# tigarcia/firedancer

Measured on AMD Instinct MI355X. Metric: ed25519 verifies/sec at 1/8 GPUs; % INT32 VALU roofline; p99 batch latency, higher is better.
Workload: dtype int32

## Files before the change

### firedancer_amd/csrc/fd25519_half.h

```cpp
#ifndef FD25519_HALF_H
#define FD25519_HALF_H

#include <stdint.h>

#ifndef FD_HALF_FN
#define FD_HALF_FN static inline
#endif

#define FD_HALF_BITS 131
#define FD_HALF_DBITS_MAX 151
#define FD_HALF_TW   5
#ifndef FD_HALF_LEHMER_MARGIN
#define FD_HALF_LEHMER_MARGIN 0
#endif

#define FD_HALF_N8L {0xe7ae9f68u, 0xc09318d2u, 0x17bce6b2u, 0xa6f7cef5u, 0u, 0u, 0u, 0x80000000u}

template <int N>
FD_HALF_FN int fd_half_bitlen(const uint32_t (&x)[N]) {
  int r = 0;
#pragma unroll
  for (int i = 0; i < N; i++)
    if (x[i]) r = 32 * i + 32 - __builtin_clz(x[i]);
  return r;
}

FD_HALF_FN uint64_t fd_half_shr64(const uint32_t (&x)[8], int s) {
  const int w = s >> 5, sh = s & 31;
  uint32_t x0 = 0u, x1 = 0u, x2 = 0u;
#pragma unroll
  for (int i = 0; i < 8; i++) {
    x0 = i == w ? x[i] : x0;
    x1 = i == w + 1 ? x[i] : x1;
    x2 = i == w + 2 ? x[i] : x2;
  }
  const uint64_t lo = (((uint64_t)x1 << 32) | x0) >> sh;
  const uint64_t hi = (((uint64_t)x2 << 32) | x1) >> sh;
  return (lo & 0xffffffffu) | (hi << 32);
}

FD_HALF_FN int fd_half_lt(const uint32_t (&a)[8], const uint32_t (&b)[8]) {
  int r = 0;
#pragma unroll
  for (int i = 0; i < 8; i++) r = a[i] != b[i] ? (a[i] < b[i]) : r;
  return r;
}

template <int N>
FD_HALF_FN void fd_half_mul_small(uint32_t (&out)[N], const uint32_t (&x)[N], uint64_t m) {
  const uint64_t m0 = m & 0xffffffffu, m1 = m >> 32;
  uint64_t c = 0;
#pragma unroll
  for (int i = 0; i < N; i++) {
    const uint64_t t = (uint64_t)x[i] * m0 + c;
    out[i] = (uint32_t)t;
    c = t >> 32;
  }
  c = 0;
#pragma unroll
  for (int i = 0; i + 1 < N; i++) {
    const uint64_t t = (uint64_t)x[i] * m1 + out[i + 1] + c;
    out[i + 1] = (uint32_t)t;
    c = t >> 32;
  }
}

template <int N>
FD_HALF_FN void fd_half_lin(uint32_t (&out)[N], const uint32_t (&x)[N], const uint32_t (&y)[N], int64_t A,
                            int64_t B) {
  uint32_t px[N], py[N];
  fd_half_mul_small<N>(px, x, (uint64_t)(A < 0 ? -A : A));
  fd_half_mul_small<N>(py, y, (uint64_t)(B < 0 ? -B : B));
  const uint32_t fx = A < 0 ? 0xffffffffu : 0u, fy = B < 0 ? 0xffffffffu : 0u;
  uint64_t c = (uint64_t)(A < 0) + (uint64_t)(B < 0);
#pragma unroll
  for (int i = 0; i < N; i++) {
    const uint64_t t = (uint64_t)(px[i] ^ fx) + (uint64_t)(py[i] ^ fy) + c;
    out[i] = (uint32_t)t;
    c = t >> 32;
  }
}

FD_HALF_FN void fd_half_step(uint32_t (&a)[8], const uint32_t (&b)[8], uint32_t (&ta)[FD_HALF_TW],
                             const uint32_t (&tb)[FD_HALF_TW], uint64_t q) {
  uint32_t p[8], pt[FD_HALF_TW];
  fd_half_mul_small<8>(p, b, q);
  fd_half_mul_small<FD_HALF_TW>(pt, tb, q);
  uint64_t br = 0;
#pragma unroll
  for (int i = 0; i < 8; i++) {
    const uint64_t t = (uint64_t)a[i] - p[i] - br;
    a[i] = (uint32_t)t;
    br = (t >> 63) & 1u;
  }
  br = 0;
#pragma unroll
  for (int i = 0; i < FD_HALF_TW; i++) {
    const uint64_t t = (uint64_t)ta[i] - pt[i] - br;
    ta[i] = (uint32_t)t;
    br = (t >> 63) & 1u;
  }
}

FD_HALF_FN uint64_t fd_half_quot(const uint32_t (&a)[8], const uint32_t (&b)[8]) {
  const int la = fd_half_bitlen<8>(a);
  const int s = la > 52 ? la - 52 : 0;
  const uint64_t ah = fd_half_shr64(a, s), bh = fd_half_shr64(b, s);
  const double r = (double)ah / (double)(bh + 1u) * (1.0 - 0x1p-40);
  const uint64_t q = (uint64_t)r;
  return q ? q : 1u;
}

FD_HALF_FN void fd_half_swap(uint32_t (&a)[8], uint32_t (&b)[8], uint32_t (&ta)[FD_HALF_TW],
                             uint32_t (&tb)[FD_HALF_TW], int cond) {
#pragma unroll
  for (int i = 0; i < 8; i++) {
    const uint32_t x = a[i], y = b[i];
    a[i] = cond ? y : x;
    b[i] = cond ? x : y;
  }
#pragma unroll
  for (int i = 0; i < FD_HALF_TW; i++) {
    const uint32_t x = ta[i], y = tb[i];
    ta[i] = cond ? y : x;
    tb[i] = cond ? x : y;
  }
}

FD_HALF_FN void fd_half_single(uint32_t (&a)[8], uint32_t (&b)[8], uint32_t (&ta)[FD_HALF_TW],
                               uint32_t (&tb)[FD_HALF_TW]) {
  fd_half_step(a, b, ta, tb, fd_half_quot(a, b));
  fd_half_swap(a, b, ta, tb, fd_half_lt(a, b));
}

#ifndef FD_HALF_RCP
#define FD_HALF_RCP(y) (1.0 / (y))
#endif
FD_HALF_FN double fd_half_fdiv(double x, double y) {
  double r = FD_HALF_RCP(y);
  r = __builtin_fma(r, __builtin_fma(-y, r, 1.0), r);
  double q = __builtin_floor(x * r);
#pragma unroll
  for (int i = 0; i < 2; i++) {
    const double rem = __builtin_fma(-q, y, x);
    q = rem < 0.0 ? q - 1.0 : (rem >= y ? q + 1.0 : q);
  }
  return q;
}

#ifndef FD_HALF_RCPF
#define FD_HALF_RCPF(y) (1.0f / (y))
#endif
FD_HALF_FN double fd_half_fdiv32(double x, double y) {
  double q = __builtin_floor((double)((float)x * FD_HALF_RCPF((float)y)));
  double rem = __builtin_fma(-q, y, x);
  q = rem < 0.0 ? q - 1.0 : (rem >= y ? q + 1.0 : q);
  rem = __builtin_fma(-q, y, x);
  return (rem >= 0.0 && rem < y) ? q : -1.0;
}

FD_HALF_FN double fd_half_fdiv20(double x, double y) {
  const double e = (double)((float)x * FD_HALF_RCPF((float)y));
  double q = __builtin_floor(e);
  const double rem = __builtin_fma(-q, y, x);
  q = rem < 0.0 ? q - 1.0 : (rem >= y ? q + 1.0 : q);
  return e < 0x1p20 ? q : -1.0;
}

#ifndef FD_HALF_INNER
#define FD_HALF_INNER 4
#endif
#if FD_HALF_INNER >= 3
#define FD_HALF_QUOT(x, y) fd_half_fdiv20((x), (y))
#elif FD_HALF_INNER == 2
#define FD_HALF_QUOT(x, y) fd_half_fdiv32((x), (y))
#else
#define FD_HALF_QUOT(x, y) fd_half_fdiv((x), (y))
#endif

FD_HALF_FN int fd_half_abs(uint32_t (&mag)[FD_HALF_TW], const uint32_t (&x)[FD_HALF_TW]) {
  const int neg = (int)(x[FD_HALF_TW - 1] >> 31);
  const uint32_t f = neg ? 0xffffffffu : 0u;
  uint64_t c = (uint64_t)neg;
#pragma unroll
  for (int i = 0; i < FD_HALF_TW; i++) {
    const uint64_t t = (uint64_t)(x[i] ^ f) + c;
    mag[i] = (uint32_t)t;
    c = t >> 32;
  }
  return neg;
}

FD_HALF_FN int fd_half_scalars(const uint32_t (&k)[8], uint32_t (&c)[FD_HALF_TW], uint32_t (&dmag)[FD_HALF_TW],
                               int* dneg, int dbits) {
  uint32_t a[8] = FD_HALF_N8L, b[8];
  uint32_t ta[FD_HALF_TW] = {0u, 0u, 0u, 0u, 0u}, tb[FD_HALF_TW] = {1u, 0u, 0u, 0u, 0u};
#pragma unroll
  for (int i = 0; i < 8; i++) b[i] = k[i];
  int ok = 1, it = 0;

  while (fd_half_bitlen<8>(b) > FD_HALF_BITS + FD_HALF_LEHMER_MARGIN) {
    if (++it > 200) { ok = 0; break; }
    const int s = fd_half_bitlen<8>(a) - 52;
    double uh = (double)fd_half_shr64(a, s), vh = (double)fd_half_shr64(b, s);
    const int fl = FD_HALF_BITS + FD_HALF_LEHMER_MARGIN - s;
    const double floor_v = fl > 0 ? (double)((uint64_t)1 << (fl < 62 ? fl : 62)) : 0.0;
    double Af = 1.0, Bf = 0.0, Cf = 0.0, Df = 1.0;
    for (int inner = 0; inner < 64; inner++) {
      const double x1 = uh + Af, y1 = vh + Cf, x2 = uh + Bf, y2 = vh + Df;
#if FD_HALF_INNER == 0
      if (!(y1 > 0.0 && y2 > 0.0 && x1 >= 0.0 && x2 >= 0.0)) break;
      const double q = fd_half_fdiv(x1, y1);
      if (q != fd_half_fdiv(x2, y2)) break;
      const double nv = __builtin_fma(-q, vh, uh);
      if (nv < floor_v) break;
#elif FD_HALF_INNER == 4
      const bool valid = (y1 > 0.0) & (y2 > 0.0) & (x1 >= 0.0) & (x2 >= 0.0);
      const double q = fd_half_fdiv20(x1, y1), q2 = fd_half_fdiv20(x2, y2);
      const double nv = __builtin_fma(-q, vh, uh);
      const double nC = __builtin_fma(-q, Cf, Af), nD = __builtin_fma(-q, Df, Bf);
      const bool ok1 = valid & (q >= 0.0) & (q == q2) & (nv >= floor_v);
      const double x1b = vh + Cf, y1b = nv + nC, x2b = vh + Df, y2b = nv + nD;
      const bool validb = (y1b > 0.0) & (y2b > 0.0) & (x1b >= 0.0) & (x2b >= 0.0);
      const double qb = fd_half_fdiv20(x1b, y1b), q2b = fd_half_fdiv20(x2b, y2b);
      const double nvb = __builtin_fma(-qb, nv, vh);
      const double nCb = __builtin_fma(-qb, nC, Cf), nDb = __builtin_fma(-qb, nD, Df);
      const bool ok2 = validb & (qb >= 0.0) & (qb == q2b) & (nvb >= floor_v);
      if (!(ok1 & ok2)) {
        if (ok1) { Af = Cf; Cf = nC; Bf = Df; Df = nD; uh = vh; vh = nv; }
        break;
      }
      Af = nC; Cf = nCb; Bf = nD; Df = nDb;
      uh = nv; vh = nvb;
      inner++;
      continue;
#elif FD_HALF_INNER == 3
      const bool valid = (y1 > 0.0) & (y2 > 0.0) & (x1 >= 0.0) & (x2 >= 0.0);
      const double q = FD_HALF_QUOT(x1, y1), q2 = FD_HALF_QUOT(x2, y2);
      const double nv = __builtin_fma(-q, vh, uh);
      const double nC = __builtin_fma(-q, Cf, Af), nD = __builtin_fma(-q, Df, Bf);
      if (!(valid & (q >= 0.0) & (q == q2) & (nv >= floor_v))) break;
      Af = Cf; Cf = nC; Bf = Df; Df = nD;
      uh = vh; vh = nv;
      continue;
#else
      const bool valid = (y1 > 0.0) & (y2 > 0.0) & (x1 >= 0.0) & (x2 >= 0.0);
      const double q = FD_HALF_QUOT(x1, valid ? y1 : 1.0), q2 = FD_HALF_QUOT(x2, valid ? y2 : 1.0);
      const double nv = __builtin_fma(-q, vh, uh);
      if (!(valid & (q >= 0.0) & (q == q2) & (nv >= floor_v))) break;
#endif
      double T = __builtin_fma(-q, Cf, Af); Af = Cf; Cf = T;
      T = __builtin_fma(-q, Df, Bf); Bf = Df; Df = T;
      uh = vh; vh = nv;
    }
    const int64_t A = (int64_t)Af, B = (int64_t)Bf, C = (int64_t)Cf, D = (int64_t)Df;
    if (B == 0) {
      fd_half_single(a, b, ta, tb);
    } else {
      uint32_t na[8], nb[8], nta[FD_HALF_TW], ntb[FD_HALF_TW];
      fd_half_lin<8>(na, a, b, A, B);
      fd_half_lin<8>(nb, a, b, C, D);
      fd_half_lin<FD_HALF_TW>(nta, ta, tb, A, B);
      fd_half_lin<FD_HALF_TW>(ntb, ta, tb, C, D);
#pragma unroll
      for (int i = 0; i < 8; i++) { a[i] = na[i]; b[i] = nb[i]; }
#pragma unroll
      for (int i = 0; i < FD_HALF_TW; i++) { ta[i] = nta[i]; tb[i] = ntb[i]; }
    }
  }
  while (ok && fd_half_bitlen<8>(b) > FD_HALF_BITS) {
    if (++it > 400) { ok = 0; break; }
    fd_half_single(a, b, ta, tb);
  }
  uint32_t cw[8], dw[FD_HALF_TW];
  if (tb[0] & 1u) {
#pragma unroll
    for (int i = 0; i < 8; i++) cw[i] = b[i];
#pragma unroll
    for (int i = 0; i < FD_HALF_TW; i++) dw[i] = tb[i];
  } else {
    uint32_t x[8], dummy[FD_HALF_TW] = {0u, 0u, 0u, 0u, 0u};
    const uint32_t zt[FD_HALF_TW] = {0u, 0u, 0u, 0u, 0u};
    const int big = fd_half_bitlen<8>(a) > FD_HALF_BITS;
    uint64_t br = 0;
#pragma unroll
    for (int i = 0; i < 8; i++) {
      const uint32_t sub = i == FD_HALF_BITS / 32 ? (1u << (FD_HALF_BITS % 32)) : 0u;
      const uint64_t t = (uint64_t)a[i] - sub - br;
      x[i] = (uint32_t)t;
      br = (t >> 63) & 1u;
    }
    uint64_t m = 0;
    const int zb = fd_half_bitlen<8>(b) == 0;
    if (zb || fd_half_bitlen<8>(a) - fd_half_bitlen<8>(b) > 60) ok = 0;
    int guard = 0;
    while (ok && big && !fd_half_lt(x, b)) {
      if (++guard > 8) { ok = 0; break; }
      const uint64_t q = fd_half_quot(x, b);
      fd_half_step(x, b, dummy, zt, q);
      m += q;
    }
    if (big) m += 1;
    {
      uint32_t tm[FD_HALF_TW];
      fd_half_abs(tm, tb);
      const int mb = m ? 64 - __builtin_clzll(m) : 0;
      if (mb + fd_half_bitlen<FD_HALF_TW>(tm) > 155) ok = 0;
    }
    fd_half_lin<8>(cw, a, b, 1, -(int64_t)m);
    fd_half_lin<FD_HALF_TW>(dw, ta, tb, 1, -(int64_t)m);
  }
#pragma unroll
  for (int i = 0; i < FD_HALF_TW; i++) c[i] = cw[i];
  *dneg = fd_half_abs(dmag, dw);
  uint32_t chi = 0u;
#pragma unroll
  for (int i = FD_HALF_TW; i < 8; i++) chi |= cw[i];
  if (chi || fd_half_bitlen<FD_HALF_TW>(c) > FD_HALF_BITS || fd_half_bitlen<FD_HALF_TW>(dmag) > dbits ||
      !(dw[0] & 1u))
    ok = 0;
  return ok;
}

#endif
```

Before: 103.8 million.

## Streamline Lehmer half-GCD scalar reduction with 32-bit cofactor updates and cheaper tests

```diff
diff --git a/firedancer_amd/csrc/fd25519_half.h b/firedancer_amd/csrc/fd25519_half.h
--- a/firedancer_amd/csrc/fd25519_half.h
+++ b/firedancer_amd/csrc/fd25519_half.h
@@ -81,6 +81,46 @@
   }
 }
 
+#define FD_HALF_LIN32_MAX 0x1p30
+template <int N>
+FD_HALF_FN void fd_half_lin32(uint32_t (&out)[N], const uint32_t (&x)[N], const uint32_t (&y)[N], int32_t A,
+                              int32_t B) {
+  const uint32_t fx = A < 0 ? 0xffffffffu : 0u, fy = B < 0 ? 0xffffffffu : 0u;
+  const uint32_t ma = (uint32_t)(A < 0 ? -A : A), mb = (uint32_t)(B < 0 ? -B : B);
+  uint64_t c = (uint64_t)(ma & fx) + (uint64_t)(mb & fy);
+#pragma unroll
+  for (int i = 0; i < N; i++) {
+    const uint64_t t = (uint64_t)ma * (x[i] ^ fx) + (uint64_t)mb * (y[i] ^ fy) + c;
+    out[i] = (uint32_t)t;
+    c = t >> 32;
+  }
+}
+
+template <int BIT>
+FD_HALF_FN int fd_half_ge_pow2(const uint32_t (&x)[8]) {
+  uint32_t hi = x[BIT / 32] >> (BIT % 32);
+#pragma unroll
+  for (int i = BIT / 32 + 1; i < 8; i++) hi |= x[i];
+  return hi != 0u;
+}
+
+FD_HALF_FN int fd_half_lead52(const uint32_t (&a)[8], const uint32_t (&b)[8], double* uh, double* vh) {
+  uint32_t a2 = a[7], a1 = a[6], a0 = a[5], b2 = b[7], b1 = b[6], b0 = b[5];
+  int h = 7;
+#pragma unroll
+  for (int i = 4; i >= 2; i--) {
+    const int z = a2 == 0u;
+    a2 = z ? a1 : a2; a1 = z ? a0 : a1; a0 = z ? a[i] : a0;
+    b2 = z ? b1 : b2; b1 = z ? b0 : b1; b0 = z ? b[i] : b0;
+    h -= z;
+  }
+  const int sh = 44 - (a2 ? __builtin_clz(a2) : 32);
+  const uint64_t al = ((uint64_t)a1 << 32) | a0, bl = ((uint64_t)b1 << 32) | b0;
+  *uh = (double)(((uint64_t)a2 << (64 - sh)) | (al >> sh));
+  *vh = (double)(((uint64_t)b2 << (64 - sh)) | (bl >> sh));
+  return 32 * (h - 2) + sh;
+}
+
 FD_HALF_FN void fd_half_step(uint32_t (&a)[8], const uint32_t (&b)[8], uint32_t (&ta)[FD_HALF_TW],
                              const uint32_t (&tb)[FD_HALF_TW], uint64_t q) {
   uint32_t p[8], pt[FD_HALF_TW];
@@ -167,8 +207,17 @@
   return e < 0x1p20 ? q : -1.0;
 }
 
+FD_HALF_FN double fd_half_fdiv20u(double* q, double* r, double x, double y) {
+  const double e = (double)((float)x * FD_HALF_RCPF((float)y));
+  const double q0 = __builtin_floor(e);
+  const double rem = __builtin_fma(-q0, y, x);
+  *q = rem < 0.0 ? q0 - 1.0 : (rem >= y ? q0 + 1.0 : q0);
+  *r = __builtin_fma(-*q, y, x);
+  return e;
+}
+
 #ifndef FD_HALF_INNER
-#define FD_HALF_INNER 4
+#define FD_HALF_INNER 5
 #endif
 #if FD_HALF_INNER >= 3
 #define FD_HALF_QUOT(x, y) fd_half_fdiv20((x), (y))
@@ -178,6 +227,11 @@
 #define FD_HALF_QUOT(x, y) fd_half_fdiv((x), (y))
 #endif
 
+#ifndef FD_HALF_HOOK_STEP
+#define FD_HALF_HOOK_ROUND(a, b) ((void)0)
+#define FD_HALF_HOOK_STEP(q) ((void)0)
+#endif
+
 FD_HALF_FN int fd_half_abs(uint32_t (&mag)[FD_HALF_TW], const uint32_t (&x)[FD_HALF_TW]) {
   const int neg = (int)(x[FD_HALF_TW - 1] >> 31);
   const uint32_t f = neg ? 0xffffffffu : 0u;
@@ -199,16 +253,40 @@
   for (int i = 0; i < 8; i++) b[i] = k[i];
   int ok = 1, it = 0;
 
-  while (fd_half_bitlen<8>(b) > FD_HALF_BITS + FD_HALF_LEHMER_MARGIN) {
+  while (fd_half_ge_pow2<FD_HALF_BITS + FD_HALF_LEHMER_MARGIN>(b)) {
     if (++it > 200) { ok = 0; break; }
-    const int s = fd_half_bitlen<8>(a) - 52;
-    double uh = (double)fd_half_shr64(a, s), vh = (double)fd_half_shr64(b, s);
+    FD_HALF_HOOK_ROUND(a, b);
+    double uh, vh;
+    const int s = fd_half_lead52(a, b, &uh, &vh);
+    const double uh0 = uh, vh0 = vh;
     const int fl = FD_HALF_BITS + FD_HALF_LEHMER_MARGIN - s;
     const double floor_v = fl > 0 ? (double)((uint64_t)1 << (fl < 62 ? fl : 62)) : 0.0;
     double Af = 1.0, Bf = 0.0, Cf = 0.0, Df = 1.0;
     for (int inner = 0; inner < 64; inner++) {
       const double x1 = uh + Af, y1 = vh + Cf, x2 = uh + Bf, y2 = vh + Df;
-#if FD_HALF_INNER == 0
+#if FD_HALF_INNER == 5
+      (void)x1; (void)x2;
+      const double fv = fl > 0 ? floor_v : 1.0;
+      double q, nv, qb, nvb;
+      const double e = fd_half_fdiv20u(&q, &nv, uh, vh);
+      const double nC = __builtin_fma(-q, Cf, Af), nD = __builtin_fma(-q, Df, Bf);
+      const double s1 = nv + nC, s2 = nv + nD;
+      const bool ok1 = (e < 0x1p20) & (s1 >= fv) & (s2 >= fv) & (y1 - s1 >= 0.0) & (y2 - s2 >= 0.0);
+      const double eb = fd_half_fdiv20u(&qb, &nvb, vh, nv);
+      const double nCb = __builtin_fma(-qb, nC, Cf), nDb = __builtin_fma(-qb, nD, Df);
+      const double s1b = nvb + nCb, s2b = nvb + nDb;
+      const bool ok2 = (eb < 0x1p20) & (s1b >= fv) & (s2b >= fv) & (s1 - s1b >= 0.0) & (s2 - s2b >= 0.0);
+      if (!(ok1 & ok2)) {
+        if (ok1) { FD_HALF_HOOK_STEP(q); Af = Cf; Cf = nC; Bf = Df; Df = nD; uh = vh; vh = nv; }
+        break;
+      }
+      FD_HALF_HOOK_STEP(q);
+      FD_HALF_HOOK_STEP(qb);
+      Af = nC; Cf = nCb; Bf = nD; Df = nDb;
+      uh = nv; vh = nvb;
+      inner++;
+      continue;
+#elif FD_HALF_INNER == 0
       if (!(y1 > 0.0 && y2 > 0.0 && x1 >= 0.0 && x2 >= 0.0)) break;
       const double q = fd_half_fdiv(x1, y1);
       if (q != fd_half_fdiv(x2, y2)) break;
@@ -253,22 +331,37 @@
       T = __builtin_fma(-q, Df, Bf); Bf = Df; Df = T;
       uh = vh; vh = nv;
     }
-    const int64_t A = (int64_t)Af, B = (int64_t)Bf, C = (int64_t)Cf, D = (int64_t)Df;
-    if (B == 0) {
+    int single = 0;
+    if (Bf == 0.0) {
+      if (vh0 >= 1.0) {
+        const double ql = fd_half_fdiv(uh0, vh0 + 1.0), qu = fd_half_fdiv(uh0 + 1.0, vh0);
+        if (ql == qu) { FD_HALF_HOOK_STEP(ql); Af = 0.0; Bf = 1.0; Cf = 1.0; Df = -ql; }
+        else if (ql >= 2.0) { Af = 1.0; Bf = 1.0 - ql; Cf = 0.0; Df = 1.0; }
+        else single = 1;
+      } else {
+        single = 1;
+      }
+    }
+    const int fits = (__builtin_fabs(Af) < FD_HALF_LIN32_MAX) & (__builtin_fabs(Bf) < FD_HALF_LIN32_MAX) &
+                     (__builtin_fabs(Cf) < FD_HALF_LIN32_MAX) & (__builtin_fabs(Df) < FD_HALF_LIN32_MAX);
+    if (single | !fits) {
       fd_half_single(a, b, ta, tb);
-    } else {
-      uint32_t na[8], nb[8], nta[FD_HALF_TW], ntb[FD_HALF_TW];
-      fd_half_lin<8>(na, a, b, A, B);
-      fd_half_lin<8>(nb, a, b, C, D);
-      fd_half_lin<FD_HALF_TW>(nta, ta, tb, A, B);
-      fd_half_lin<FD_HALF_TW>(ntb, ta, tb, C, D);
-#pragma unroll
-      for (int i = 0; i < 8; i++) { a[i] = na[i]; b[i] = nb[i]; }
-#pragma unroll
-      for (int i = 0; i < FD_HALF_TW; i++) { ta[i] = nta[i]; tb[i] = ntb[i]; }
-    }
-  }
-  while (ok && fd_half_bitlen<8>(b) > FD_HALF_BITS) {
+      continue;
+    }
+    uint32_t na[8], nb[8], nta[FD_HALF_TW], ntb[FD_HALF_TW];
+    {
+      const int32_t A = (int32_t)Af, B = (int32_t)Bf, C = (int32_t)Cf, D = (int32_t)Df;
+      fd_half_lin32<8>(na, a, b, A, B);
+      fd_half_lin32<8>(nb, a, b, C, D);
+      fd_half_lin32<FD_HALF_TW>(nta, ta, tb, A, B);
+      fd_half_lin32<FD_HALF_TW>(ntb, ta, tb, C, D);
+    }
+#pragma unroll
+    for (int i = 0; i < 8; i++) { a[i] = na[i]; b[i] = nb[i]; }
+#pragma unroll
+    for (int i = 0; i < FD_HALF_TW; i++) { ta[i] = nta[i]; tb[i] = ntb[i]; }
+  }
+  while (FD_HALF_LEHMER_MARGIN > 0 && ok && fd_half_ge_pow2<FD_HALF_BITS>(b)) {
     if (++it > 400) { ok = 0; break; }
     fd_half_single(a, b, ta, tb);
   }
@@ -281,7 +374,7 @@
   } else {
     uint32_t x[8], dummy[FD_HALF_TW] = {0u, 0u, 0u, 0u, 0u};
     const uint32_t zt[FD_HALF_TW] = {0u, 0u, 0u, 0u, 0u};
-    const int big = fd_half_bitlen<8>(a) > FD_HALF_BITS;
+    const int big = fd_half_ge_pow2<FD_HALF_BITS>(a);
     uint64_t br = 0;
 #pragma unroll
     for (int i = 0; i < 8; i++) {
@@ -291,10 +384,24 @@
       br = (t >> 63) & 1u;
     }
     uint64_t m = 0;
-    const int zb = fd_half_bitlen<8>(b) == 0;
-    if (zb || fd_half_bitlen<8>(a) - fd_half_bitlen<8>(b) > 60) ok = 0;
+    const int la = fd_half_bitlen<8>(a), lb = fd_half_bitlen<8>(b);
+    if (lb == 0 || la - lb > 60) ok = 0;
+    int direct = 0;
+    if (ok && big) {
+      const int lx = fd_half_bitlen<8>(x);
+      if (lb > lx) {
+        direct = 1;
+      } else {
+        const int sx = lx > 52 ? lx - 52 : 0;
+        const double xs = (double)fd_half_shr64(x, sx), bs = (double)fd_half_shr64(b, sx);
+        if (bs >= 1.0) {
+          const double ql = fd_half_fdiv(xs, bs + 1.0), qu = fd_half_fdiv(xs + 1.0, bs);
+          if (ql == qu) { m = (uint64_t)ql; direct = 1; }
+        }
+      }
+    }
     int guard = 0;
-    while (ok && big && !fd_half_lt(x, b)) {
+    while (ok && big && !direct && !fd_half_lt(x, b)) {
       if (++guard > 8) { ok = 0; break; }
       const uint64_t q = fd_half_quot(x, b);
       fd_half_step(x, b, dummy, zt, q);
@@ -307,8 +414,13 @@
       const int mb = m ? 64 - __builtin_clzll(m) : 0;
       if (mb + fd_half_bitlen<FD_HALF_TW>(tm) > 155) ok = 0;
     }
-    fd_half_lin<8>(cw, a, b, 1, -(int64_t)m);
-    fd_half_lin<FD_HALF_TW>(dw, ta, tb, 1, -(int64_t)m);
+    if (m < (uint64_t)FD_HALF_LIN32_MAX) {
+      fd_half_lin32<8>(cw, a, b, 1, -(int32_t)m);
+      fd_half_lin32<FD_HALF_TW>(dw, ta, tb, 1, -(int32_t)m);
+    } else {
+      fd_half_lin<8>(cw, a, b, 1, -(int64_t)m);
+      fd_half_lin<FD_HALF_TW>(dw, ta, tb, 1, -(int64_t)m);
+    }
   }
 #pragma unroll
   for (int i = 0; i < FD_HALF_TW; i++) c[i] = cw[i];
```

Result: faster. 105.5 million, median of 6 (+1.6%).
